# AuroraEchos/Sound-Event-Localization-and-Detection

Measured on AMD Instinct MI355X. Metric: train-step samples/sec (8ch x 128mel x 512T), higher is better.
Workload: dtype f32; 1 GPU; c3: DQSELD-TCN-S1-PHI_8ch train step, F=128 T=512 (U=L=192, SURVEY F3), batch 32/GPU, random-init weights; global_batch=32, parallelism=dp1, step_mode=graph (auto: probe 9.57 ms recorded / 12.83 ms eager per step), deterministic=True

## Files before the change

sound-event-localization-and-detection_amd/csrc/hcq_conv.hip:

```cpp
#include <string.h>
#include <type_traits>
#include "hc_common.h"

#ifndef HCQ_DBG
#define HCQ_DBG 0
#endif
#ifndef HCQ_PIN
#define HCQ_PIN 1
#endif
#ifndef HCQ_XDMA
#define HCQ_XDMA 1
#endif

namespace seld {

struct HcqP {
    const float* src;
    const float* src2;
    int nsrc;
    int mix_ytile;
    const float* wpack;
    float* dst[2];
    const float* bias[2];
    const float* addend[2];
    float* stats[2];
    int epilogue[2];
    int A;
    int N, Csrc, Cdst;
    int IB, OB;
    int W;
    int Himg;
    int dil, dpad;
    int wext;
    int nch;
    int half_src[2];
    int ytiles;
    int ob_step;
    int tile_half[3][2];
    int tile_ob[3][2];
    long long range_stride[2];
    long long ytile_stride;
    long long set_stride;
};

typedef unsigned int uintx4h __attribute__((ext_vector_type(4)));
typedef int int4h __attribute__((ext_vector_type(4)));

__device__ __forceinline__ void hcq_dma16(unsigned lds_addr, unsigned voff, int4h rsrc) {
    unsigned keep;
    asm volatile("s_mov_b32 %0, m0\n\ts_mov_b32 m0, %1\n\ts_nop 0\n\tbuffer_load_dwordx4 %2, %3, 0 offen lds\n\ts_mov_b32 m0, %0"
                 : "=&s"(keep) : "s"(lds_addr), "v"(voff), "s"(rsrc) : "memory");
}
__device__ __forceinline__ int4h hcq_rsrc(const float* base, unsigned bytes) {
    const unsigned long long a = (unsigned long long)base;
    return (int4h){(int)(unsigned)a, (int)((unsigned)(a >> 32) & 0xFFFFu), (int)bytes, 0x00020000};
}

__device__ __forceinline__ int small_div_h(int n, float inv_d) { return (int)(((float)n + 0.5f) * inv_d); }

__device__ __forceinline__ void xforms(const float b[4], float g[8]) {
    g[0] = b[1] + b[2];
    g[1] = b[0] + b[3];
    g[2] = b[0] - b[3];
    g[3] = b[1] - b[2];
    g[4] = b[2] - b[3];
    g[5] = b[1] + b[0];
    g[6] = b[2] + b[3];
    g[7] = b[1] - b[0];
}

template <int KH, int KW, int IBC, int NT1, int NT2, int NR, int XI, bool MX = false>
__global__ __launch_bounds__(256, 2) void hcq_conv_kernel(const HcqP p) {
    constexpr int TAPS = KH * KW;
    constexpr int NT = NT1 + NT2;
    constexpr int KQ = IBC * TAPS;
    constexpr int NG = (KQ + 3) / 4;
    constexpr int NPAIR = (NG + 1) / 2;
    extern __shared__ __attribute__((aligned(16))) float lds[];

    const int tid = threadIdx.x;
    const int lane = tid & 63;
    const int wave = __builtin_amdgcn_readfirstlane(tid >> 6);
    const int fr = lane & 15, fk = lane >> 4;
    const int A = p.A;
    const int ROWS = A * IBC * KH;
    const int wext = p.wext, qw = wext >> 2;
    const int buf_floats = ROWS * wext;

    const unsigned tiles_per_row = (unsigned)p.W >> 6;
    const unsigned bx = (gridDim.x & 7u) ? blockIdx.x : (blockIdx.x & 7u) * (gridDim.x >> 3) + (blockIdx.x >> 3);
    const unsigned row_g = bx / tiles_per_row;
    const int w0 = (int)(bx - row_g * tiles_per_row) * 64;
    const int n_img = (int)(row_g / (unsigned)p.Himg);
    const int h0 = (int)row_g - n_img * p.Himg;
    const int yt = blockIdx.y;
    const int set = yt >= p.ytiles ? 1 : 0;
    const int ytile = yt - set * p.ytiles;
    const bool mix_wg = ytile == p.mix_ytile;

    const unsigned S = (unsigned)(p.Himg * p.W);
    const unsigned src_bytes = (unsigned)p.N * (unsigned)p.Csrc * S * 4u;
    const unsigned OOB = 0xFFFFFFF0u;
    __amdgpu_buffer_rsrc_t rsrc = __builtin_amdgcn_make_buffer_rsrc((void*)p.src, 0, src_bytes, 0x00020000);
    unsigned xoff[XI];
    int xlds[XI];
    const unsigned xadv = (unsigned)IBC * S * 4u;
    const int total_items = ROWS * qw;
    {
        int row = small_div_h(tid, 1.0f / (float)qw);
        int quad = tid - row * qw;
        const int drow = 256 / qw, dquad = 256 - drow * qw;
        const unsigned img_base = (unsigned)n_img * (unsigned)p.Csrc * S;
#pragma unroll
        for (int i = 0; i < XI; ++i) {
            const bool in = tid + 256 * i < total_items;
            const int kh = row % KH;
            const int ci = row / KH;
            const int comp = ci / IBC;
            const int ibl = ci - comp * IBC;
            const int hh = h0 + (kh - (KH - 1) / 2);
            const int ww = w0 - p.dpad + 4 * quad;
            const bool ok = in && (unsigned)hh < (unsigned)p.Himg && (unsigned)ww < (unsigned)p.W;
            const unsigned e = img_base + ((unsigned)(comp * p.IB + ibl) * (unsigned)p.Himg + (unsigned)hh) * (unsigned)p.W + (unsigned)ww;
            xoff[i] = ok ? e * 4u : OOB;
            xlds[i] = in ? (row * qw + quad) * 4 : -1;
            row += drow;
            quad += dquad;
            if (quad >= qw) { quad -= qw; ++row; }
        }
    }
#if HCQ_XDMA
    const unsigned lds0 = (unsigned)(size_t)(__attribute__((address_space(3))) unsigned char*)lds;
    int4h xrs = hcq_rsrc(p.src, src_bytes);
    int xchunk = 0;
    int xbuf = 0;
    auto load_x = [&]() __attribute__((always_inline)) {
        if (xchunk == p.nch) {
            xrs = hcq_rsrc(p.src2, src_bytes);
#pragma unroll
            for (int i = 0; i < XI; ++i) xoff[i] = xoff[i] == OOB ? OOB : xoff[i] - (unsigned)p.nch * xadv;
        }
        ++xchunk;
        const unsigned base = lds0 + (unsigned)xbuf * (unsigned)buf_floats * 4u + 1024u * (unsigned)wave;
#pragma unroll
        for (int i = 0; i < XI; ++i) {
            if (xlds[i] >= 0) hcq_dma16(base + 4096u * (unsigned)i, xoff[i], xrs);
            xoff[i] = xoff[i] == OOB ? OOB : xoff[i] + xadv;
        }
        xbuf ^= 1;
    };
    auto store_x = [&](int) __attribute__((always_inline)) { asm volatile("s_waitcnt vmcnt(0)" ::: "memory"); };
#else
    floatx4 xr[XI];
    int xchunk = 0;
    auto load_x = [&]() __attribute__((always_inline)) {
        if (xchunk == p.nch) {
            rsrc = __builtin_amdgcn_make_buffer_rsrc((void*)p.src2, 0, src_bytes, 0x00020000);
#pragma unroll
            for (int i = 0; i < XI; ++i) xoff[i] = xoff[i] == OOB ? OOB : xoff[i] - (unsigned)p.nch * xadv;
        }
        ++xchunk;
#pragma unroll
        for (int i = 0; i < XI; ++i) {
            const uintx4h v = __builtin_amdgcn_raw_buffer_load_b128(rsrc, xoff[i], 0, 0);
            xr[i][0] = __uint_as_float(v[0]); xr[i][1] = __uint_as_float(v[1]);
            xr[i][2] = __uint_as_float(v[2]); xr[i][3] = __uint_as_float(v[3]);
            xoff[i] = xoff[i] == OOB ? OOB : xoff[i] + xadv;
        }
    };
    auto store_x = [&](int buf) __attribute__((always_inline)) {
        float* b = lds + buf * buf_floats;
#pragma unroll
        for (int i = 0; i < XI; ++i)
            if (xlds[i] >= 0) *reinterpret_cast<float4*>(b + xlds[i]) = make_float4(xr[i][0], xr[i][1], xr[i][2], xr[i][3]);
    };
#endif

    int aoff[NG];
#pragma unroll
    for (int g = 0; g < NG; ++g) {
        const int kq = (4 * g + fk) < KQ ? 4 * g + fk : 0;
        const int ibl = kq / TAPS;
        const int tap = kq - ibl * TAPS;
        const int kh = tap / KW;
        const int kw = tap - kh * KW;
        aoff[g] = (ibl * KH + kh) * wext + p.dpad + wave * 16 + fr + (kw - (KW - 1) / 2) * p.dil;
    }
    const int comp_stride = IBC * KH * wext;

    const float* wbase = p.wpack + (long long)set * p.set_stride + (long long)ytile * p.ytile_stride;
    const long long chunk_stride = p.range_stride[0] + (NR > 1 ? p.range_stride[1] : 0);

    floatx4 acc[NT][8];
#pragma unroll
    for (int t = 0; t < NT; ++t)
#pragma unroll
        for (int m = 0; m < 8; ++m) acc[t][m] = (floatx4){0.f, 0.f, 0.f, 0.f};

    float2 bfr[8][NT];
    float gm[2][8];
    float raw[4];
    constexpr int NPC = NR * NPAIR;

    bool dbg_started = false;
    auto load_b1 = [&](const float* blk, int j, int m, auto ntrc, auto t0c) __attribute__((always_inline)) {
        constexpr int NTR = decltype(ntrc)::value, T0 = decltype(t0c)::value;
        if ((HCQ_DBG & 1) && dbg_started) return;
        const float* q = blk + ((long long)(j * 8 + m) * 64 + lane) * (2 * NTR);
#pragma unroll
        for (int t = T0; t < NTR; ++t) bfr[m][t] = *reinterpret_cast<const float2*>(q + 2 * t);
    };
    auto read_raw = [&](const float* xs, int g) __attribute__((always_inline)) {
        if ((HCQ_DBG & 2) && dbg_started) return;
#pragma unroll
        for (int q = 0; q < 4; ++q) raw[q] = xs[aoff[g] + q * comp_stride];
    };
    using I0 = std::integral_constant<int, 0>;
    using INT = std::integral_constant<int, NT>;
    using INT1 = std::integral_constant<int, NT1>;
    using INT2 = std::integral_constant<int, NT2>;

    const int nchunks = p.nch * p.nsrc;
    auto kloop = [&](auto mixc) __attribute__((always_inline)) {
    constexpr bool MIX = decltype(mixc)::value;
    using IT0 = std::integral_constant<int, MIX ? NT1 : 0>;
    load_x();
    store_x(0);
#pragma unroll
    for (int m = 0; m < 8; ++m) load_b1(wbase, 0, m, INT{}, IT0{});
    __syncthreads();
    for (int ch = 0; ch < nchunks; ++ch) {
        const int buf = ch & 1;
        if (ch + 1 < nchunks && !(HCQ_DBG & 4)) load_x();
        const float* xb = lds + buf * buf_floats;
        const float* wc = wbase + (long long)ch * chunk_stride;
        const bool more = ch + 1 < nchunks;
        const float* wn = wc + chunk_stride;
        const float* xs0 = xb + p.half_src[0] * 4 * comp_stride;
        const float* xs1 = xb + p.half_src[1] * 4 * comp_stride;
        read_raw(xs0, 0);
        if (!(HCQ_DBG & 2) || !dbg_started) xforms(raw, gm[0]);
        if ((HCQ_DBG & 2) && !dbg_started) xforms(raw, gm[1]);
        dbg_started = true;
#pragma unroll
        for (int s = 0; s < NR * NG; ++s) {
            const int r = s / NG, g = s - r * NG;
            const int pc = r * NPAIR + g / 2;
            const int gst = s & 1;
            const bool last = s + 1 == NR * NG;
            const bool pair_ends = (g & 1) == 1 || g + 1 == NG;
            if (!last) {
                const int rn = (s + 1) / NG, gn = (s + 1) - rn * NG;
                read_raw(rn == 0 ? xs0 : xs1, gn);
            }
            __builtin_amdgcn_sched_barrier(0);
#pragma unroll
            for (int m = 0; m < 8; ++m) {
                if (r == 0) {
#pragma unroll
                    for (int t = MIX ? NT1 : 0; t < NT; ++t)
                        acc[t][m] = __builtin_amdgcn_mfma_f32_16x16x4f32(gm[gst][m], (g & 1) ? bfr[m][t].y : bfr[m][t].x,
                                                                          acc[t][m], 0, 0, 0);
                } else {
#pragma unroll
                    for (int t = 0; t < NT2; ++t)
                        acc[NT1 + t][m] = __builtin_amdgcn_mfma_f32_16x16x4f32(gm[gst][m], (g & 1) ? bfr[m][t].y : bfr[m][t].x,
                                                                                acc[NT1 + t][m], 0, 0, 0);
                }
                if (pair_ends) {
                    const int pn = pc + 1;
                    if (pn < NPC) {
                        const int rn = pn / NPAIR, jn = pn - rn * NPAIR;
                        if (rn == 0) load_b1(wc, jn, m, INT{}, IT0{});
                        else load_b1(wc + p.range_stride[0], jn, m, INT2{}, I0{});
                    } else if (more) {
                        load_b1(wn, 0, m, INT{}, IT0{});
                    }
                    if (HCQ_PIN && (NT >= 3 || HCQ_XDMA)) __builtin_amdgcn_sched_barrier(0);
                }
            }
            if (!last && !(HCQ_DBG & 2)) xforms(raw, gm[gst ^ 1]);
            __builtin_amdgcn_sched_barrier(0);
        }
        if (ch + 1 < nchunks && !(HCQ_DBG & 4)) store_x(buf ^ 1);
        if (!(HCQ_DBG & 8)) __syncthreads();
    }
    };
    if constexpr (MX) {
        static_assert(NR == 2 && NT1 == 1 && NT2 == 1, "the only layout with mixed-tile workgroups");
        if (mix_wg) kloop(std::true_type{});
        else kloop(std::false_type{});
    } else {
        kloop(std::false_type{});
    }

    float* const dst = p.dst[set];
    const float* const bias = p.bias[set];
    const float* const addend = p.addend[set];
    float* const stats = p.stats[set];
    const int epi = p.epilogue[set];
    const int grp = fr >> 3;
    const unsigned pos_off = (unsigned)h0 * (unsigned)p.W + (unsigned)(w0 + wave * 16 + fk * 4);
    const unsigned img_off = (unsigned)n_img * (unsigned)p.Cdst * S;
    float* redbuf = lds;
    auto epilogue = [&](auto plainc) __attribute__((always_inline)) {
        constexpr bool PLAIN = decltype(plainc)::value;
#pragma unroll
        for (int t = 0; t < NT; ++t) {
            const int ds = mix_wg ? 2 : t;
            const int ob0 = (mix_wg && t != NT1) ? -1 : p.tile_ob[ds][grp];
            const int half = p.tile_half[ds][grp];
            const bool chok = ob0 >= 0;
            const int ob = (chok ? ob0 : 0) + (mix_wg ? 0 : ytile * p.ob_step) + (fr & 7);
            floatx4 c[4];
#pragma unroll
            for (int r = 0; r < 4; ++r) {
                const float h0_ = 0.5f * acc[t][0][r], h1 = 0.5f * acc[t][1][r], h2 = 0.5f * acc[t][2][r], h3 = 0.5f * acc[t][3][r];
                c[0][r] = (h3 - h0_) + (h1 + h2) + acc[t][4][r];
                c[1][r] = (h3 - h0_) - (h1 + h2) + acc[t][5][r];
                c[2][r] = (h3 + h0_) + (h2 - h1) + acc[t][6][r];
                c[3][r] = (h3 + h0_) + (h1 - h2) - acc[t][7][r];
            }
#pragma unroll
            for (int q = 0; q < 4; ++q) {
                const int chn = (half * 4 + q) * p.OB + ob;
                const unsigned off = img_off + (unsigned)chn * S + pos_off;
                if (PLAIN) {
                    if (chok) *reinterpret_cast<float4*>(dst + off) = make_float4(c[q][0], c[q][1], c[q][2], c[q][3]);
                    continue;
                }
                float s1 = 0.f, s2 = 0.f;
                if (chok) {
                    const float bv = bias ? bias[chn] : 0.f;
                    float4 o = make_float4(c[q][0] + bv, c[q][1] + bv, c[q][2] + bv, c[q][3] + bv);
                    if (epi & SELD_EPI_ADD) {
                        const float4 ad = *reinterpret_cast<const float4*>(addend + off);
                        o.x += ad.x; o.y += ad.y; o.z += ad.z; o.w += ad.w;
                    }
                    if (epi & SELD_EPI_ACCUMULATE) {
                        const float4 old = *reinterpret_cast<const float4*>(dst + off);
                        o.x += old.x; o.y += old.y; o.z += old.z; o.w += old.w;
                    }
                    *reinterpret_cast<float4*>(dst + off) = o;
                    s1 = o.x + o.y + o.z + o.w;
                    s2 = o.x * o.x + o.y * o.y + o.z * o.z + o.w * o.w;
                }
                if (epi & SELD_EPI_STATS) {
                    s1 += __shfl_xor(s1, 16, 64);
                    s1 += __shfl_xor(s1, 32, 64);
                    s2 += __shfl_xor(s2, 16, 64);
                    s2 += __shfl_xor(s2, 32, 64);
                    if (fk == 0) {
                        const int slot = ((wave * NT + t) * 4 + q) * 16 + fr;
                        redbuf[slot * 2 + 0] = s1;
                        redbuf[slot * 2 + 1] = s2;
                    }
                }
            }
        }
    };
    if (epi == 0 && !bias) epilogue(std::true_type{});
    else epilogue(std::false_type{});
    if (epi & SELD_EPI_STATS) {
        __syncthreads();
        float* rep = stats + (size_t)(blockIdx.x % SELD_STATS_REPLICAS) * 2 * p.Cdst;
        for (int e = tid; e < NT * 4 * 16; e += 256) {
            const int fr_ = e & 15, q = (e >> 4) & 3, t = e >> 6;
            const int g_ = fr_ >> 3;
            const int ds = mix_wg ? 2 : t;
            const int ob0 = (mix_wg && t != NT1) ? -1 : p.tile_ob[ds][g_];
            if (ob0 < 0) continue;
            const int chn = (p.tile_half[ds][g_] * 4 + q) * p.OB + ob0 + (mix_wg ? 0 : ytile * p.ob_step) + (fr_ & 7);
            float a1 = 0.f, a2 = 0.f;
#pragma unroll
            for (int wv = 0; wv < 4; ++wv) {
                const int slot = ((wv * NT + t) * 4 + q) * 16 + fr_;
                a1 += redbuf[slot * 2 + 0];
                a2 += redbuf[slot * 2 + 1];
            }
            atomicAdd(rep + chn, a1);
            atomicAdd(rep + p.Cdst + chn, a2);
        }
    }
}

template <int IBC, int NT1, int NT2, int NR, int R>
__global__ __launch_bounds__(256, 2) void hcq_first_kernel(const HcqP p) {
    constexpr int KH = 3, KW = 3, TAPS = 9;
    constexpr int NT = NT1 + NT2;
    constexpr int KQ = IBC * TAPS;
    constexpr int NG = (KQ + 3) / 4;
    constexpr int NPAIR = (NG + 1) / 2;
    constexpr int NPC = NR * NPAIR;
    constexpr int XR = R + KH - 1;
    extern __shared__ __attribute__((aligned(16))) float lds[];

    const int tid = threadIdx.x;
    const int lane = tid & 63;
    const int wave = __builtin_amdgcn_readfirstlane(tid >> 6);
    const int fr = lane & 15, fk = lane >> 4;
    const int A = p.A;
    constexpr int wext = 72, qw = wext >> 2, DPAD = 4;

    const unsigned tiles_per_row = (unsigned)p.W >> 6;
    const unsigned hblocks = (unsigned)p.Himg / R;
    unsigned b = blockIdx.x;
    if ((gridDim.x & 7u) == 0) b = (blockIdx.x & 7u) * (gridDim.x >> 3) + (blockIdx.x >> 3);
    const int w0 = (int)(b % tiles_per_row) * 64;
    b /= tiles_per_row;
    const int h0 = (int)(b % hblocks) * R;
    const int n_img = (int)(b / hblocks);

    const unsigned S = (unsigned)(p.Himg * p.W);
    {
        const unsigned src_bytes = (unsigned)p.N * (unsigned)p.Csrc * S * 4u;
        const unsigned OOB = 0xFFFFFFF0u;
        const __amdgpu_buffer_rsrc_t rsrc = __builtin_amdgcn_make_buffer_rsrc((void*)p.src, 0, src_bytes, 0x00020000);
        const int items = A * IBC * XR * qw;
        const unsigned img_base = (unsigned)n_img * (unsigned)p.Csrc * S;
        constexpr float inv_qw = 1.0f / (float)qw;
        for (int f0 = tid; f0 < items; f0 += 4 * 256) {
            uintx4h v[4];
            int dst_[4];
#pragma unroll
            for (int u = 0; u < 4; ++u) {
                const int f = f0 + 256 * u;
                const int row = small_div_h(f, inv_qw);
                const int quad = f - row * qw;
                const int ci = row / XR;
                const int xr = row - ci * XR;
                const int comp = ci / IBC;
                const int ibl = ci - comp * IBC;
                const int hh = h0 - (KH - 1) / 2 + xr;
                const int ww = w0 - DPAD + 4 * quad;
                const bool ok = f < items && (unsigned)hh < (unsigned)p.Himg && (unsigned)ww < (unsigned)p.W;
                const unsigned e = img_base + ((unsigned)(comp * p.IB + ibl) * (unsigned)p.Himg + (unsigned)hh) * (unsigned)p.W + (unsigned)ww;
                v[u] = __builtin_amdgcn_raw_buffer_load_b128(rsrc, ok ? e * 4u : OOB, 0, 0);
                dst_[u] = f < items ? (row * qw + quad) * 4 : -1;
            }
#pragma unroll
            for (int u = 0; u < 4; ++u)
                if (dst_[u] >= 0)
                    *reinterpret_cast<float4*>(lds + dst_[u]) =
                        make_float4(__uint_as_float(v[u][0]), __uint_as_float(v[u][1]), __uint_as_float(v[u][2]), __uint_as_float(v[u][3]));
        }
    }
// ... 401 lines not shown
            for (int q = 0; q < 4; ++q) {
                float a1 = s1[q], a2 = s2[q];
                a1 += __shfl_xor(a1, 16, 64);
                a1 += __shfl_xor(a1, 32, 64);
                a2 += __shfl_xor(a2, 16, 64);
                a2 += __shfl_xor(a2, 32, 64);
                if (fk == 0) {
                    const int slot = ((T * 4 + wave) * 4 + q) * 16 + fr;
                    sred[slot * 2 + 0] = a1;
                    sred[slot * 2 + 1] = a2;
                }
            }
        }
    };
    tile_body(std::integral_constant<int, 0>{});
    if constexpr (NT > 1) tile_body(std::integral_constant<int, 1>{});
    if constexpr (NT > 2) tile_body(std::integral_constant<int, 2>{});

    if (want_stats) {
        __syncthreads();
        float* rep = p.stats[0] + (size_t)(blockIdx.x % SELD_STATS_REPLICAS) * 2 * p.Cdst;
        for (int e = tid; e < NT * 4 * 16; e += 256) {
            const int fr_ = e & 15, q = (e >> 4) & 3, t = e >> 6;
            const int g_ = fr_ >> 3;
            const int ob0 = p.tile_ob[t][g_];
            if (ob0 < 0) continue;
            const int chn = (p.tile_half[t][g_] * 4 + q) * p.OB + ob0 + (fr_ & 7);
            float a1 = 0.f, a2 = 0.f;
#pragma unroll
            for (int wv = 0; wv < 4; ++wv) {
                const int slot = ((t * 4 + wv) * 4 + q) * 16 + fr_;
                a1 += sred[slot * 2 + 0];
                a2 += sred[slot * 2 + 1];
            }
            atomicAdd(rep + chn, a1);
            atomicAdd(rep + p.Cdst + chn, a2);
        }
    }
}

struct HcqPackP {
    WPtrs w[2];
    float* out;
    int A, mode;
    int OA, IA, taps;
    int IBC, nch, NR, NT1, NT2, NG, NPAIR;
    int half_src[2];
    int nreg;
    int has_mix;
    int nsets;
    int nsrc;
    int ob_step;
    int tile_half[3][2], tile_ob[3][2];
    long long range_stride[2], ytile_stride, set_stride, total;
};

__device__ __forceinline__ float hcq_pack_value(const HcqPackP& p, long long idx) {
    const int NT = p.NT1 + p.NT2;
    const unsigned set_stride = (unsigned)p.set_stride, ytile_stride = (unsigned)p.ytile_stride;
    const unsigned set = (unsigned)idx / set_stride;
    unsigned r0 = (unsigned)idx - set * set_stride;
    const int ytile = (int)(r0 / ytile_stride);
    r0 -= (unsigned)ytile * ytile_stride;
    const bool mix = p.has_mix && ytile == p.nreg;
    const unsigned rs[2] = {(unsigned)p.range_stride[0], (unsigned)p.range_stride[1]};
    const unsigned chunk_stride = rs[0] + (p.NR > 1 ? rs[1] : 0);
    const int chs = (int)(r0 / chunk_stride);
    r0 -= (unsigned)chs * chunk_stride;
    const int srcsel = chs / p.nch, ch = chs - srcsel * p.nch;
    const int range = (r0 >= rs[0]) ? 1 : 0;
    if (range) r0 -= rs[0];
    const int ntr = range ? p.NT2 : NT;
    const int per_m = 64 * 2 * ntr;
    const int per_pair = 8 * per_m;
    const int j = (int)(r0 / (unsigned)per_pair);
    int r1 = (int)(r0 - (unsigned)j * (unsigned)per_pair);
    const int m = r1 / per_m;
    r1 -= m * per_m;
    const int lane = r1 / (2 * ntr);
    r1 -= lane * 2 * ntr;
    const int t = r1 >> 1, gg = r1 & 1;
    const int k = lane >> 4, n = lane & 15;
    const int g = 2 * j + gg;
    if (g >= p.NG) return 0.f;
    const int kq = 4 * g + k;
    if (kq >= p.IBC * p.taps) return 0.f;
    const int tf = range ? p.NT1 + t : t;
    const int ds = mix ? 2 : tf;
    const int grp = n >> 3;
    const int ob0 = (mix && tf != p.NT1) ? -1 : p.tile_ob[ds][grp];
    if (ob0 < 0) return 0.f;
    const int dblk = ob0 + (mix ? 0 : ytile * p.ob_step) + (n & 7);
    const int kbl = kq / p.taps;
    const int tap = kq - kbl * p.taps;
    const int sblk = ch * p.IBC + kbl;
    const int hd = p.tile_half[ds][grp], hs = p.half_src[range];
    int qsel = 0;
    if (p.A == 8) {
        if (p.mode == 0) qsel = (hd == hs) ? 0 : (hd == 1 ? 1 : -1);
        else qsel = (hd == hs) ? 0 : (hd == 0 ? 1 : -1);
    }
    if (qsel < 0) return 0.f;
    const int co = p.mode == 0 ? dblk : sblk;
    const int ci = p.mode == 0 ? sblk : dblk;
    const int tp = p.mode == 0 ? tap : p.taps - 1 - tap;
    if (co >= p.OA || ci >= p.IA) return 0.f;
    const size_t e = ((size_t)co * p.IA + ci) * p.taps + tp;
    const WPtrs& w = p.w[p.mode == 0 ? set : srcsel];
    float a[4];
#pragma unroll
    for (int c = 0; c < 4; ++c) a[c] = w.p[qsel * 4 + c][e];
    if (p.mode == 1) { a[1] = -a[1]; a[2] = -a[2]; a[3] = -a[3]; }
    switch (m) {
        case 0: return a[3] + a[1];
        case 1: return a[0] - a[2];
        case 2: return a[0] + a[2];
        case 3: return a[3] - a[1];
        case 4: return a[3] - a[2];
        case 5: return a[1] + a[0];
        case 6: return a[0] - a[1];
        default: return a[3] + a[2];
    }
}

__global__ __launch_bounds__(256) void hcq_pack_kernel(const HcqPackP p) {
    const long long idx = (long long)blockIdx.x * 256 + threadIdx.x;
    if (idx < p.total) p.out[idx] = hcq_pack_value(p, idx);
}

__global__ __launch_bounds__(256) void hcq_pack_flat_kernel(const HcqPackP* __restrict__ table, const int* __restrict__ starts,
                                                            int nentries) {
    const int b = blockIdx.x;
    int lo = 0, hi = nentries;
    while (hi - lo > 1) {
        const int mid = (lo + hi) >> 1;
        if (starts[mid] <= b) lo = mid; else hi = mid;
    }
    const HcqPackP& p = table[lo];
    const long long idx = (long long)(b - starts[lo]) * 256 + threadIdx.x;
    if (idx < p.total) p.out[idx] = hcq_pack_value(p, idx);
}

__global__ __launch_bounds__(256) void hcq_pack_table_kernel(const HcqPackP* __restrict__ table, int nentries) {
    const int e = blockIdx.y;
    if (e >= nentries) return;
    const HcqPackP& p = table[e];
    for (long long idx = (long long)blockIdx.x * 256 + threadIdx.x; idx < p.total; idx += (long long)gridDim.x * 256)
        p.out[idx] = hcq_pack_value(p, idx);
}

struct HcqPlan {
    int ok;
    int KH, KW, IBC, NT1, NT2, NR, XI, mix;
    int first_rows;
    HcqP kp;
    HcqPackP pp;
    size_t pack_floats;
    dim3 grid;
    size_t smem;
};

static HcqPlan hcq_plan(const seld_conv_desc* d, int mode, int npair) {
    HcqPlan pl{};
    const bool pool = mode == 2;
    if (pool) mode = 0;
    const int A = d->algebra;
    if (A != 4 && A != 8) return pl;
    if (d->stride[0] != 1 || d->stride[1] != 1 || d->dil[0] != 1) return pl;
    int o[2];
    hc_out_shape(d, o);
    if (o[0] != d->in[0] || o[1] != d->in[1]) return pl;
    const int KH = d->k[0], KW = d->k[1];
    if (!((KH == 1 && (KW == 1 || KW == 3)) || (KH == 3 && KW == 3))) return pl;
    if (2 * d->pad[1] != d->dil[1] * (KW - 1) || 2 * d->pad[0] != (KH - 1)) return pl;
    if (KW == 1 && d->dil[1] != 1) return pl;
    const int W = d->in[1], Himg = d->in[0];
    if (W % 64) return pl;
    const int Csrc = mode == 0 ? d->Cin : d->Cout, Cdst = mode == 0 ? d->Cout : d->Cin;
    const int IB = Csrc / A, OB = Cdst / A;
    if ((long long)d->N * Csrc * Himg * W * 4 >= 0xFFFFFFF0ll || (long long)d->N * Cdst * Himg * W * 4 >= 0xFFFFFFF0ll) return pl;
    const int taps = KH * KW;
    const int nsets = mode == 0 ? npair : 1, nsrc = mode == 1 ? npair : 1;
    const int dil = KW == 3 ? d->dil[1] : 0;
    const int dpad = KW == 3 ? (dil + 3) / 4 * 4 : 0;
    const int wext = 64 + 2 * dpad;
    static const int cand11[] = {16, 24, 8, 0}, cand13[] = {8, 4, 0}, cand33[] = {4, 2, 1, 0};
    const int* cand = taps == 1 ? cand11 : (taps == 3 ? cand13 : cand33);
    int IBC = 0;
    size_t smem = 0;
    for (int i = 0; cand[i]; ++i) {
        if (IB % cand[i]) continue;
        const int nbuf = (IB / cand[i]) * nsrc > 1 ? 2 : 1;
        const size_t need = (size_t)nbuf * A * cand[i] * KH * wext * sizeof(float);
        if (need <= 78 * 1024) { IBC = cand[i]; smem = need; break; }
    }
    if (!IBC) return pl;
    if (!pool && mode == 0 && taps == 9 && A == 8 && IB == 1 && Cdst == 192 && (long long)d->N * Himg * W >= 256 * 128 &&
        !env().conv_no_smallk) return pl;
    const int rows = A * IBC * KH;
    const int items = rows * (wext / 4);
    const int XI = (items + 255) / 256;
    if (smem < 8 * 1024) smem = 8 * 1024;
    HcqP& k = pl.kp;
    int NT1, NT2, NR, nreg, ob_step, mix = 0;
    for (int t = 0; t < 3; ++t)
        for (int g = 0; g < 2; ++g) { k.tile_half[t][g] = 0; k.tile_ob[t][g] = -1; }
    if (A == 8) {
        NR = 2;
        const int both = mode == 0 ? 1 : 0;
        const int once = 1 - both;
        k.half_src[0] = mode == 0 ? 0 : 1;
        k.half_src[1] = 1 - k.half_src[0];
        if (OB % 16 != 0 && OB % 16 != 8) return pl;
        NT1 = 1; NT2 = 1; nreg = OB / 16; ob_step = 16;
        k.tile_half[0][0] = k.tile_half[0][1] = once; k.tile_ob[0][0] = 0; k.tile_ob[0][1] = 8;
        k.tile_half[1][0] = k.tile_half[1][1] = both; k.tile_ob[1][0] = 0; k.tile_ob[1][1] = 8;
        if (OB % 16 == 8) {
            k.tile_half[2][0] = once; k.tile_ob[2][0] = OB - 8;
            k.tile_half[2][1] = both; k.tile_ob[2][1] = OB - 8;
            const long long ptiles = (long long)d->N * Himg * W / 64;
            if (OB == 24 && ptiles * nsets >= 512) { NT2 = 2; ob_step = 0; }
            else mix = 1;
        }
        if (nreg == 0) return pl;
    } else {
        NR = 1; NT2 = 0;
        k.half_src[0] = k.half_src[1] = 0;
        if (OB % 32 == 0) { NT1 = 2; nreg = OB / 32; ob_step = 32; }
        else if (OB % 16 == 0) { NT1 = 1; nreg = OB / 16; ob_step = 16; }
        else return pl;
        for (int t = 0; t < NT1; ++t) { k.tile_ob[t][0] = 16 * t; k.tile_ob[t][1] = 16 * t + 8; }
    }
    const int NG = (IBC * taps + 3) / 4, NPAIR = (NG + 1) / 2;
    const int NT = NT1 + NT2;
    k.A = A; k.N = d->N; k.Csrc = Csrc; k.Cdst = Cdst; k.IB = IB; k.OB = OB;
    k.W = W; k.Himg = Himg; k.dil = dil; k.dpad = dpad; k.wext = wext; k.nch = IB / IBC;
    k.nsrc = nsrc;
    k.ytiles = nreg + mix; k.mix_ytile = mix ? nreg : -1; k.ob_step = ob_step;
    k.range_stride[0] = (long long)NPAIR * 8 * 64 * 2 * NT;
    k.range_stride[1] = (long long)NPAIR * 8 * 64 * 2 * NT2;
    k.ytile_stride = (long long)nsrc * k.nch * (k.range_stride[0] + (NR > 1 ? k.range_stride[1] : 0));
    k.set_stride = (long long)(nreg + mix) * k.ytile_stride;
    pl.pack_floats = (size_t)k.set_stride * nsets;
    HcqPackP& q = pl.pp;
    q.A = A; q.mode = mode; q.OA = d->Cout / A; q.IA = d->Cin / A; q.taps = taps;
    q.IBC = IBC; q.nch = k.nch; q.NR = NR; q.NT1 = NT1; q.NT2 = NT2; q.NG = NG; q.NPAIR = NPAIR;
    q.half_src[0] = k.half_src[0]; q.half_src[1] = k.half_src[1];
    q.nreg = nreg; q.has_mix = mix; q.nsets = nsets; q.nsrc = nsrc; q.ob_step = ob_step;
    for (int t = 0; t < 3; ++t)
        for (int g = 0; g < 2; ++g) { q.tile_half[t][g] = k.tile_half[t][g]; q.tile_ob[t][g] = k.tile_ob[t][g]; }
    q.range_stride[0] = k.range_stride[0]; q.range_stride[1] = k.range_stride[1];
    q.ytile_stride = k.ytile_stride; q.set_stride = k.set_stride; q.total = (long long)pl.pack_floats;
    pl.KH = KH; pl.KW = KW; pl.IBC = IBC; pl.NT1 = NT1; pl.NT2 = NT2; pl.NR = NR; pl.XI = XI; pl.mix = mix;
    const long long ptot = (long long)d->N * Himg * W;
    pl.grid = dim3((unsigned)(ptot / 64), (unsigned)(k.ytiles * nsets), 1);
    pl.smem = smem;
    constexpr int FIRST_R = 8;
    if (mode == 0 && taps == 9 && IBC == IB && IB <= 2 && k.ytiles == 1 && nsets == 1 && !mix && Himg % FIRST_R == 0 && wext == 72) {
        pl.first_rows = FIRST_R;
        pl.grid = dim3((unsigned)(ptot / 64 / FIRST_R), 1, 1);
        pl.smem = ((size_t)A * IBC * (FIRST_R + 2) * wext + 4 * NT * 4 * 64 * 2) * sizeof(float);
    }
    if (pool && !pl.first_rows) return HcqPlan{};
    pl.ok = 1;
    return pl;
}

struct HcqKern { int KH, KW, IBC, NT1, NT2, NR, XI; };
static int hcq_pick(const HcqPlan& pl, HcqKern* k) {
    int xi8 = 0, xi4 = 0;
    if (pl.KH == 1 && pl.KW == 3 && pl.IBC == 8) {
        xi8 = pl.XI <= 5 ? 5 : (pl.XI <= 7 ? 7 : 9);
        xi4 = pl.XI <= 3 ? 3 : 5;
    } else if (pl.KH == 1 && pl.KW == 3 && pl.IBC == 4) { xi8 = 6; xi4 = 3; }
    else if (pl.KH == 1 && pl.KW == 1 && pl.IBC == 16) { xi8 = 8; xi4 = 4; }
    else if (pl.KH == 1 && pl.KW == 1 && pl.IBC == 24) { xi8 = 12; xi4 = 6; }
    else if (pl.KH == 1 && pl.KW == 1 && pl.IBC == 8) { xi8 = 4; xi4 = 2; }
    else if (pl.KH == 3 && pl.KW == 3 && pl.IBC == 4) { xi8 = 7; xi4 = 4; }
    else if (pl.KH == 3 && pl.KW == 3 && pl.IBC == 2) { xi8 = 4; xi4 = 2; }
    else if (pl.KH == 3 && pl.KW == 3 && pl.IBC == 1) { xi8 = 2; xi4 = 1; }
    else return 0;
    const int xi = pl.NR == 2 ? xi8 : xi4;
    if (pl.XI > xi) return 0;
    *k = HcqKern{pl.KH, pl.KW, pl.IBC, pl.NT1, pl.NT2, pl.NR, xi};
    return 1;
}

template <int KH, int KW, int IBC, int NT1, int NT2, int NR, int XI, bool MX = false>
static int hcq_launch_one(const HcqPlan& pl, hipStream_t st) {
    auto kern = hcq_conv_kernel<KH, KW, IBC, NT1, NT2, NR, XI, MX>;
    if (pl.smem > 64 * 1024 &&
        hipFuncSetAttribute((const void*)kern, hipFuncAttributeMaxDynamicSharedMemorySize, (int)pl.smem) != hipSuccess)
        return SELD_ELAUNCH;
    hipLaunchKernelGGL(kern, pl.grid, dim3(256), pl.smem, st, pl.kp);
    return check_launch();
}

template <int KH, int KW, int IBC, int XI8, int XI4>
static int hcq_launch_cfg(const HcqPlan& pl, const HcqKern& k, hipStream_t st) {
    if (k.NR == 2) {
        if (k.XI != XI8) return SELD_EUNSUPPORTED;
        if (k.NT2 == 2) return hcq_launch_one<KH, KW, IBC, 1, 2, 2, XI8>(pl, st);
        if (pl.mix) return hcq_launch_one<KH, KW, IBC, 1, 1, 2, XI8, true>(pl, st);
        return hcq_launch_one<KH, KW, IBC, 1, 1, 2, XI8>(pl, st);
    }
    if (k.XI != XI4) return SELD_EUNSUPPORTED;
    return k.NT1 == 2 ? hcq_launch_one<KH, KW, IBC, 2, 0, 1, XI4>(pl, st)
                      : hcq_launch_one<KH, KW, IBC, 1, 0, 1, XI4>(pl, st);
}

template <int IBC, int NT1, int NT2, int NR>
static int hcq_launch_first(const HcqPlan& pl, hipStream_t st) {
    auto kern = hcq_first_kernel<IBC, NT1, NT2, NR, 8>;
    if (pl.smem > 64 * 1024 &&
        hipFuncSetAttribute((const void*)kern, hipFuncAttributeMaxDynamicSharedMemorySize, (int)pl.smem) != hipSuccess)
        return SELD_ELAUNCH;
    hipLaunchKernelGGL(kern, pl.grid, dim3(256), pl.smem, st, pl.kp);
    return check_launch();
}

static bool hcq_first_takes(const HcqPlan& pl) {
    if (!pl.first_rows || pl.first_rows != 8) return false;
    if (pl.kp.epilogue[0] & ~SELD_EPI_STATS) return false;
    if (pl.NR == 2) return pl.NT1 == 1 && (pl.NT2 == 2 || pl.NT2 == 1);
    return pl.NT2 == 0 && (pl.NT1 == 1 || pl.NT1 == 2);
}

static int hcq_launch(const HcqPlan& pl, hipStream_t st) {
    HcqKern k;
    if (!hcq_pick(pl, &k)) return SELD_EUNSUPPORTED;
    if (hcq_first_takes(pl)) {
        if (k.IBC == 1) {
            if (k.NR == 2) return k.NT2 == 2 ? hcq_launch_first<1, 1, 2, 2>(pl, st) : hcq_launch_first<1, 1, 1, 2>(pl, st);
            return k.NT1 == 2 ? hcq_launch_first<1, 2, 0, 1>(pl, st) : hcq_launch_first<1, 1, 0, 1>(pl, st);
        }
        if (k.NR == 2) return k.NT2 == 2 ? hcq_launch_first<2, 1, 2, 2>(pl, st) : hcq_launch_first<2, 1, 1, 2>(pl, st);
        return k.NT1 == 2 ? hcq_launch_first<2, 2, 0, 1>(pl, st) : hcq_launch_first<2, 1, 0, 1>(pl, st);
    }
    if (k.KW == 3 && k.KH == 1 && k.IBC == 8) {
        if (k.NR == 2) {
            if (k.XI == 5) return hcq_launch_cfg<1, 3, 8, 5, 3>(pl, k, st);
            if (k.XI == 7) return hcq_launch_cfg<1, 3, 8, 7, 3>(pl, k, st);
            return hcq_launch_cfg<1, 3, 8, 9, 3>(pl, k, st);
        }
        if (k.XI == 3) return hcq_launch_cfg<1, 3, 8, 5, 3>(pl, k, st);
        return hcq_launch_cfg<1, 3, 8, 7, 5>(pl, k, st);
    }
    if (k.KH == 1 && k.KW == 3) return hcq_launch_cfg<1, 3, 4, 6, 3>(pl, k, st);
    if (k.KH == 1 && k.IBC == 16) return hcq_launch_cfg<1, 1, 16, 8, 4>(pl, k, st);
    if (k.KH == 1 && k.IBC == 24) return hcq_launch_cfg<1, 1, 24, 12, 6>(pl, k, st);
    if (k.KH == 1 && k.IBC == 8) return hcq_launch_cfg<1, 1, 8, 4, 2>(pl, k, st);
    if (k.IBC == 2) return hcq_launch_cfg<3, 3, 2, 4, 2>(pl, k, st);
    if (k.IBC == 1) return hcq_launch_cfg<3, 3, 1, 2, 1>(pl, k, st);
    return hcq_launch_cfg<3, 3, 4, 7, 4>(pl, k, st);
}

}

using namespace seld;

extern "C" size_t seld_hcq_pack_floats(const seld_conv_desc* d, int32_t mode, int32_t npair) {
    if (hc_validate(d) != SELD_OK || mode < 0 || mode > 2 || npair < 1 || npair > 2) return 0;
    if (env().conv_no_hcq) return 0;
    const HcqPlan pl = hcq_plan(d, mode, npair);
    HcqKern k;
    return (pl.ok && hcq_pick(pl, &k)) ? pl.pack_floats : 0;
}

extern "C" size_t seld_hcq_pack_entry_bytes(void) { return sizeof(HcqPackP); }

extern "C" int seld_hcq_kernel_label(const seld_conv_desc* d, int32_t mode, int32_t npair, char* buf, int32_t buflen) {
    if (hc_validate(d) != SELD_OK || !buf || buflen < 64) return SELD_EINVAL;
    const HcqPlan pl = hcq_plan(d, mode, npair);
    HcqKern k;
    if (!pl.ok || !hcq_pick(pl, &k)) return SELD_EUNSUPPORTED;
    if (mode == 2)
        snprintf(buf, buflen, "hcq_first_pool_kernel<%d, %d, %d, %d, 8>", k.IBC, k.NT1, k.NT2, k.NR);
    else if (pl.first_rows && hcq_first_takes(pl))
        snprintf(buf, buflen, "hcq_first_kernel<%d, %d, %d, %d, %d>", k.IBC, k.NT1, k.NT2, k.NR, pl.first_rows);
    else
        snprintf(buf, buflen, "hcq_conv_kernel<%d, %d, %d, %d, %d, %d, %d, %s>", k.KH, k.KW, k.IBC, k.NT1, k.NT2, k.NR, k.XI,
                 (pl.mix && k.NR == 2 && k.NT2 == 1) ? "true" : "false");
    return SELD_OK;
}

extern "C" int seld_hcq_pack_entry(const seld_conv_desc* d, int32_t mode, int32_t npair, const float* const wA[8],
                                   const float* const wB[8], float* wpack, void* entry) {
    if (hc_validate(d) != SELD_OK || !wA || !wpack || !entry) return SELD_EINVAL;
    if (mode < 0 || mode > 2 || npair < 1 || npair > 2 || (npair == 2 && !wB)) return SELD_EINVAL;
    HcqPlan pl = hcq_plan(d, mode, npair);
    if (!pl.ok) return SELD_EUNSUPPORTED;
    for (int i = 0; i < 8; ++i) {
        pl.pp.w[0].p[i] = i < d->algebra ? wA[i] : nullptr;
        pl.pp.w[1].p[i] = (npair == 2 && i < d->algebra) ? wB[i] : nullptr;
    }
    pl.pp.out = wpack;
    memcpy(entry, &pl.pp, sizeof(HcqPackP));
    return SELD_OK;
}

extern "C" int seld_hcq_pack(const seld_conv_desc* d, int32_t mode, int32_t npair, const float* const wA[8],
                             const float* const wB[8], float* wpack, void* stream) {
    HcqPackP e;
    const int rc = seld_hcq_pack_entry(d, mode, npair, wA, wB, wpack, &e);
    if (rc != SELD_OK) return rc;
    const unsigned blocks = (unsigned)((e.total + 255) / 256);
    hipLaunchKernelGGL(hcq_pack_kernel, dim3(blocks), dim3(256), 0, (hipStream_t)stream, e);
    return check_launch();
}

extern "C" int seld_hcq_pack_table(const void* table_dev, int32_t nentries, int64_t max_floats, void* stream) {
    if (!table_dev || nentries <= 0 || max_floats <= 0) return SELD_EINVAL;
    long long bx = (max_floats + 255) / 256;
    if (bx > 512) bx = 512;
    hipLaunchKernelGGL(hcq_pack_table_kernel, dim3((unsigned)bx, (unsigned)nentries), dim3(256), 0, (hipStream_t)stream,
                       (const HcqPackP*)table_dev, nentries);
    return check_launch();
}

extern "C" int seld_hcq_pack_flat(const void* table_dev, const int32_t* starts_dev, int32_t nentries, int32_t total_blocks,
                                  void* stream) {
    if (!table_dev || !starts_dev || nentries <= 0 || total_blocks <= 0) return SELD_EINVAL;
    hipLaunchKernelGGL(hcq_pack_flat_kernel, dim3((unsigned)total_blocks), dim3(256), 0, (hipStream_t)stream,
                       (const HcqPackP*)table_dev, starts_dev, nentries);
    return check_launch();
}

extern "C" int seld_hcq_conv(const seld_conv_desc* d, int32_t mode, int32_t npair, const float* x, const float* x2,
                             const float* wpack, float* const y[2], const float* const bias[2],
                             const int32_t epilogue[2], const float* const addend[2], float* const stats[2],
                             void* stream) {
    if (hc_validate(d) != SELD_OK || !x || !wpack || !y || !y[0]) return SELD_EINVAL;
    if ((mode != 0 && mode != 1) || npair < 1 || npair > 2) return SELD_EINVAL;
    if (mode == 1 && npair == 2 && !x2) return SELD_EINVAL;
    HcqPlan pl = hcq_plan(d, mode, npair);
    if (!pl.ok) return SELD_EUNSUPPORTED;
    const int nsets = mode == 0 ? npair : 1;
    for (int s = 0; s < 2; ++s) {
        const bool on = s < nsets;
        pl.kp.dst[s] = on ? y[s] : nullptr;
        pl.kp.bias[s] = (on && bias) ? bias[s] : nullptr;
        pl.kp.epilogue[s] = (on && epilogue) ? epilogue[s] : 0;
        pl.kp.addend[s] = (on && addend) ? addend[s] : nullptr;
        pl.kp.stats[s] = (on && stats) ? stats[s] : nullptr;
        if (on && !pl.kp.dst[s]) return SELD_EINVAL;
        if ((pl.kp.epilogue[s] & SELD_EPI_ADD) && !pl.kp.addend[s]) return SELD_EINVAL;
        if ((pl.kp.epilogue[s] & SELD_EPI_STATS) && !pl.kp.stats[s]) return SELD_EINVAL;
    }
    pl.kp.src = x;
    pl.kp.src2 = x2;
    pl.kp.wpack = wpack;
    return hcq_launch(pl, (hipStream_t)stream);
}


static int hcq_first_pool_impl(const seld_conv_desc* d, const float* x, const float* wpack, const float* bias,
                               int32_t want_stats, float* y, float* stats, const HcqPoolP& pp, bool fin, void* stream) {
    HcqPlan pl = hcq_plan(d, 2, 1);
    HcqKern k;
    if (!pl.ok || !hcq_pick(pl, &k) || pl.first_rows != 8) return SELD_EUNSUPPORTED;
    pl.kp.src = x; pl.kp.src2 = nullptr; pl.kp.wpack = wpack;
    pl.kp.dst[0] = y; pl.kp.bias[0] = bias; pl.kp.epilogue[0] = want_stats ? SELD_EPI_STATS : 0; pl.kp.stats[0] = stats;
    const int NT = pl.NT1 + pl.NT2;
    const int npair = ((pl.IBC * 9 + 3) / 4 + 1) / 2;
    const size_t smem = ((size_t)pl.kp.A * pl.IBC * 10 * 72 + (size_t)NT * 4 * 4 * 16 * 2 +
                         (size_t)pl.NR * npair * 8 * 64 * 2) * sizeof(float);
    hipStream_t st = (hipStream_t)stream;
#define SELD_FP(IBC_, NT1_, NT2_, NR_)                                                                                  \
    do {                                                                                                                \
        auto kern = fin ? hcq_first_pool_kernel<IBC_, NT1_, NT2_, NR_, 8, false, true>                                  \
                        : (y ? hcq_first_pool_kernel<IBC_, NT1_, NT2_, NR_, 8, true> : hcq_first_pool_kernel<IBC_, NT1_, NT2_, NR_, 8, false>); \
        if (smem > 64 * 1024 &&                                                                                         \
            hipFuncSetAttribute((const void*)kern, hipFuncAttributeMaxDynamicSharedMemorySize, (int)smem) != hipSuccess) \
            return SELD_ELAUNCH;                                                                                        \
        hipLaunchKernelGGL(kern, pl.grid, dim3(256), smem, st, pl.kp, pp);                                              \
        return check_launch();                                                                                          \
    } while (0)
    if (k.IBC == 1) {
        if (k.NR == 2) { if (k.NT2 == 2) SELD_FP(1, 1, 2, 2); else SELD_FP(1, 1, 1, 2); }
        if (k.NT1 == 2) SELD_FP(1, 2, 0, 1); else SELD_FP(1, 1, 0, 1);
    }
    if (k.NR == 2) { if (k.NT2 == 2) SELD_FP(2, 1, 2, 2); else SELD_FP(2, 1, 1, 2); }
    if (k.NT1 == 2) SELD_FP(2, 2, 0, 1); else SELD_FP(2, 1, 0, 1);
#undef SELD_FP
}

extern "C" int seld_hcq_first_pool(const seld_conv_desc* d, const float* x, const float* wpack, const float* bias,
                                   const float* gamma, int32_t want_stats, float* y, float* stats, float* pool_raw,
                                   uint8_t* idx, void* stream) {
    if (hc_validate(d) != SELD_OK || !x || !wpack || !gamma || !pool_raw || !idx || (want_stats && (!stats || !y))) return SELD_EINVAL;
    const HcqPoolP pp{gamma, pool_raw, idx, nullptr, nullptr, nullptr, nullptr, DropP{0.f, 1.f, 0, 0, nullptr}};
    return hcq_first_pool_impl(d, x, wpack, bias, want_stats, y, stats, pp, false, stream);
}

extern "C" int seld_hcq_first_pool_bn(const seld_conv_desc* d, const float* x, const float* wpack, const float* bias,
                                      const float* gamma, const float* beta, const float* mean, const float* invstd,
                                      float drop_p, uint64_t seed, uint64_t offset, const uint64_t* state, float* pool_raw,
                                      uint8_t* idx, float* out, void* stream) {
    if (hc_validate(d) != SELD_OK || !x || !wpack || !gamma || !beta || !mean || !invstd || !pool_raw || !idx || !out ||
        drop_p < 0.f || drop_p >= 1.f)
        return SELD_EINVAL;
    const HcqPoolP pp{gamma, pool_raw, idx, beta, mean, invstd, out, DropP{drop_p, 1.0f / (1.0f - drop_p), seed, offset, state}};
    return hcq_first_pool_impl(d, x, wpack, bias, 0, nullptr, nullptr, pp, true, stream);
}
```

Measured before the change: 3648 samples/s.

## Stage conv weight fragments through an LDS DMA ring instead of global loads

Adds a kring main loop that streams packed weight tiles into a double-buffered LDS ring with buffer_load...lds DMA. MFMA operands are then read from LDS instead of being fetched per lane from global memory. The planner sizes the ring as whole or half slots so workgroup occupancy is preserved, and falls back to the old global-fetch loop (GF) for A==4, KH==1 or when occupancy would drop. It also removes the non-DMA x-load path. The cost is extra LDS use, more barriers, and a more complex wait/barrier schedule.

```diff
diff --git a/sound-event-localization-and-detection_amd/csrc/hcq_conv.hip b/sound-event-localization-and-detection_amd/csrc/hcq_conv.hip
--- a/sound-event-localization-and-detection_amd/csrc/hcq_conv.hip
+++ b/sound-event-localization-and-detection_amd/csrc/hcq_conv.hip
@@ -7,9 +7,6 @@
 #endif
 #ifndef HCQ_PIN
 #define HCQ_PIN 1
-#endif
-#ifndef HCQ_XDMA
-#define HCQ_XDMA 1
 #endif
 
 namespace seld {
@@ -41,6 +38,8 @@
     long long range_stride[2];
     long long ytile_stride;
     long long set_stride;
+    int ring_off;
+    int half_slots;
 };
 
 typedef unsigned int uintx4h __attribute__((ext_vector_type(4)));
@@ -69,7 +68,7 @@
     g[7] = b[1] - b[0];
 }
 
-template <int KH, int KW, int IBC, int NT1, int NT2, int NR, int XI, bool MX = false>
+template <int KH, int KW, int IBC, int NT1, int NT2, int NR, int XI, bool MX = false, bool GF = false>
 __global__ __launch_bounds__(256, 2) void hcq_conv_kernel(const HcqP p) {
     constexpr int TAPS = KH * KW;
     constexpr int NT = NT1 + NT2;
@@ -101,7 +100,6 @@
     const unsigned S = (unsigned)(p.Himg * p.W);
     const unsigned src_bytes = (unsigned)p.N * (unsigned)p.Csrc * S * 4u;
     const unsigned OOB = 0xFFFFFFF0u;
-    __amdgpu_buffer_rsrc_t rsrc = __builtin_amdgcn_make_buffer_rsrc((void*)p.src, 0, src_bytes, 0x00020000);
     unsigned xoff[XI];
     int xlds[XI];
     const unsigned xadv = (unsigned)IBC * S * 4u;
@@ -129,7 +127,6 @@
             if (quad >= qw) { quad -= qw; ++row; }
         }
     }
-#if HCQ_XDMA
     const unsigned lds0 = (unsigned)(size_t)(__attribute__((address_space(3))) unsigned char*)lds;
     int4h xrs = hcq_rsrc(p.src, src_bytes);
     int xchunk = 0;
@@ -150,31 +147,6 @@
         xbuf ^= 1;
     };
     auto store_x = [&](int) __attribute__((always_inline)) { asm volatile("s_waitcnt vmcnt(0)" ::: "memory"); };
-#else
-    floatx4 xr[XI];
-    int xchunk = 0;
-    auto load_x = [&]() __attribute__((always_inline)) {
-        if (xchunk == p.nch) {
-            rsrc = __builtin_amdgcn_make_buffer_rsrc((void*)p.src2, 0, src_bytes, 0x00020000);
-#pragma unroll
-            for (int i = 0; i < XI; ++i) xoff[i] = xoff[i] == OOB ? OOB : xoff[i] - (unsigned)p.nch * xadv;
-        }
-        ++xchunk;
-#pragma unroll
-        for (int i = 0; i < XI; ++i) {
-            const uintx4h v = __builtin_amdgcn_raw_buffer_load_b128(rsrc, xoff[i], 0, 0);
-            xr[i][0] = __uint_as_float(v[0]); xr[i][1] = __uint_as_float(v[1]);
-            xr[i][2] = __uint_as_float(v[2]); xr[i][3] = __uint_as_float(v[3]);
-            xoff[i] = xoff[i] == OOB ? OOB : xoff[i] + xadv;
-        }
-    };
-    auto store_x = [&](int buf) __attribute__((always_inline)) {
-        float* b = lds + buf * buf_floats;
-#pragma unroll
-        for (int i = 0; i < XI; ++i)
-            if (xlds[i] >= 0) *reinterpret_cast<float4*>(b + xlds[i]) = make_float4(xr[i][0], xr[i][1], xr[i][2], xr[i][3]);
-    };
-#endif
 
     int aoff[NG];
 #pragma unroll
@@ -276,7 +248,7 @@
                     } else if (more) {
                         load_b1(wn, 0, m, INT{}, IT0{});
                     }
-                    if (HCQ_PIN && (NT >= 3 || HCQ_XDMA)) __builtin_amdgcn_sched_barrier(0);
+                    if (HCQ_PIN) __builtin_amdgcn_sched_barrier(0);
                 }
             }
             if (!last && !(HCQ_DBG & 2)) xforms(raw, gm[gst ^ 1]);
@@ -285,13 +257,143 @@
         if (ch + 1 < nchunks && !(HCQ_DBG & 4)) store_x(buf ^ 1);
         if (!(HCQ_DBG & 8)) __syncthreads();
     }
+    };
+
+    auto kring = [&](auto mixc) __attribute__((always_inline)) {
+    constexpr bool MIX = decltype(mixc)::value;
+    const bool half = p.half_slots != 0;
+    const unsigned tile_bytes = half ? 2048u : 4096u;
+    const unsigned slot_bytes = tile_bytes * NT;
+    const unsigned ring0 = lds0 + (unsigned)p.ring_off;
+    const float* const ringf = lds + (p.ring_off >> 2);
+    const int4h frs = hcq_rsrc(wbase, (unsigned)p.ytile_stride * 4u);
+    unsigned foff = 1024u * (unsigned)wave + 16u * (unsigned)lane;
+    unsigned fslot = 0;
+    unsigned rslot = 0;
+    bool freq = false;
+    const bool xfull = 256 * (XI - 1) + 64 * wave < total_items;
+    auto load_f = [&](auto ntrc) __attribute__((always_inline)) {
+        constexpr int NTRn = decltype(ntrc)::value;
+        const unsigned nbytes = tile_bytes * NTRn;
+        if (!((HCQ_DBG & 1) && freq)) {
+            const unsigned dst = ring0 + fslot * slot_bytes + 1024u * (unsigned)wave;
+#pragma unroll
+            for (int i = 0; i < NTRn; ++i)
+                if (4096u * i + 1024u * (unsigned)wave < nbytes) hcq_dma16(dst + 4096u * i, foff + 4096u * i, frs);
+        }
+        freq = true;
+        foff += nbytes;
+        fslot ^= 1u;
+    };
+    auto open_unit = [&](bool counted) __attribute__((always_inline)) {
+        if (counted) asm volatile("s_waitcnt vmcnt(%0)" :: "n"(XI) : "memory");
+        else asm volatile("s_waitcnt vmcnt(0)" ::: "memory");
+        if (HCQ_DBG & 8) return;
+        asm volatile("s_waitcnt lgkmcnt(0)\n\ts_barrier" ::: "memory");
+    };
+    float ga[8], gb[8];
+    float2 fb[3][NT];
+    load_x();
+    load_f(INT{});
+    bool dbg_raw = false;
+    for (int ch = 0; ch < nchunks; ++ch) {
+        const bool more = ch + 1 < nchunks;
+        const float* xb = lds + (ch & 1) * buf_floats;
+        const float* xs0 = xb + p.half_src[0] * 4 * comp_stride;
+        const float* xs1 = xb + p.half_src[1] * 4 * comp_stride;
+        bool xreq = false;
+#pragma unroll
+        for (int pc = 0; pc < NPC; ++pc) {
+            const int r = pc / NPAIR, j = pc - r * NPAIR;
+            const int g0 = 2 * j;
+            const bool two = g0 + 1 < NG;
+            const int ntr = r == 0 ? NT : NT2;
+            const int t0 = (r == 0 && MIX) ? NT1 : 0;
+            const int ab = r == 0 ? 0 : NT1;
+            auto request_next_pair = [&]() __attribute__((always_inline)) {
+                if (pc + 1 < NPC) {
+                    if ((pc + 1) / NPAIR == 0) load_f(INT{});
+                    else load_f(INT2{});
+                } else if (more) {
+                    load_f(INT{});
+                }
+            };
+            open_unit(pc == 1 && !half && xreq && xfull);
+            if (half) {
+                if (r == 0) load_f(INT{});
+                else load_f(INT2{});
+            } else {
+                request_next_pair();
+            }
+            if (pc == 0 && more && !((HCQ_DBG & 4) && ch > 0)) { load_x(); xreq = true; }
+            const float* fsl = ringf + rslot * (slot_bytes >> 2);
+            auto read_form = [&](int idx, int st) __attribute__((always_inline)) {
+                const float2* q = reinterpret_cast<const float2*>(fsl) + (idx * 64 + lane) * ntr;
+#pragma unroll
+                for (int t = 0; t < NT; ++t)
+                    if (t >= t0 && t < ntr) fb[st][t] = q[t];
+            };
+            read_form(0, 0);
+            read_form(1, 1);
+            if (!((HCQ_DBG & 2) && dbg_raw)) {
+                float ra[4], rb[4];
+                const float* xs = r == 0 ? xs0 : xs1;
+#pragma unroll
+                for (int q = 0; q < 4; ++q) ra[q] = xs[aoff[g0] + q * comp_stride];
+                if (two) {
+#pragma unroll
+                    for (int q = 0; q < 4; ++q) rb[q] = xs[aoff[two ? g0 + 1 : g0] + q * comp_stride];
+                }
+                xforms(ra, ga);
+                if (two) xforms(rb, gb);
+                dbg_raw = true;
+            }
+            __builtin_amdgcn_sched_barrier(0);
+#pragma unroll
+            for (int m = 0; m < 8; ++m) {
+                if (m == 4 && half) {
+                    open_unit(pc == 0 && xreq && xfull);
+                    request_next_pair();
+                    rslot ^= 1u;
+                    fsl = ringf + rslot * (slot_bytes >> 2);
+                    read_form(0, 4 % 3);
+                    read_form(1, 5 % 3);
+                }
+                if (m + 2 < 8) {
+                    if (m + 2 < 4 || m >= 4) read_form(half ? (m + 2) & 3 : m + 2, (m + 2) % 3);
+                    else if (!half) read_form(m + 2, (m + 2) % 3);
+                }
+                __builtin_amdgcn_sched_barrier(0);
+#pragma unroll
+                for (int t = 0; t < NT; ++t)
+                    if (t >= t0 && t < ntr)
+                        acc[ab + t][m] = __builtin_amdgcn_mfma_f32_16x16x4f32(ga[m], fb[m % 3][t].x, acc[ab + t][m], 0, 0, 0);
+                if (two) {
+#pragma unroll
+                    for (int t = 0; t < NT; ++t)
+                        if (t >= t0 && t < ntr)
+                            acc[ab + t][m] = __builtin_amdgcn_mfma_f32_16x16x4f32(gb[m], fb[m % 3][t].y, acc[ab + t][m], 0, 0, 0);
+                }
+                __builtin_amdgcn_sched_barrier(0);
+            }
+            rslot ^= 1u;
+            if (HCQ_DBG & 1) rslot = 0;
+        }
+    }
+    if (p.epilogue[set] & SELD_EPI_STATS) __syncthreads();
     };
     if constexpr (MX) {
         static_assert(NR == 2 && NT1 == 1 && NT2 == 1, "the only layout with mixed-tile workgroups");
-        if (mix_wg) kloop(std::true_type{});
-        else kloop(std::false_type{});
+        if constexpr (GF) {
+            if (mix_wg) kloop(std::true_type{});
+            else kloop(std::false_type{});
+        } else {
+            if (mix_wg) kring(std::true_type{});
+            else kring(std::false_type{});
+        }
     } else {
-        kloop(std::false_type{});
+        if constexpr (GF) kloop(std::false_type{});
+        else kring(std::false_type{});
     }
 
     float* const dst = p.dst[set];
@@ -999,6 +1101,7 @@
 struct HcqPlan {
     int ok;
     int KH, KW, IBC, NT1, NT2, NR, XI, mix;
+    int gf;
     int first_rows;
     HcqP kp;
     HcqPackP pp;
@@ -1044,10 +1147,6 @@
     if (!IBC) return pl;
     if (!pool && mode == 0 && taps == 9 && A == 8 && IB == 1 && Cdst == 192 && (long long)d->N * Himg * W >= 256 * 128 &&
         !env().conv_no_smallk) return pl;
-    const int rows = A * IBC * KH;
-    const int items = rows * (wext / 4);
-    const int XI = (items + 255) / 256;
-    if (smem < 8 * 1024) smem = 8 * 1024;
     HcqP& k = pl.kp;
     int NT1, NT2, NR, nreg, ob_step, mix = 0;
     for (int t = 0; t < 3; ++t)
@@ -1078,8 +1177,27 @@
         else return pl;
         for (int t = 0; t < NT1; ++t) { k.tile_ob[t][0] = 16 * t; k.tile_ob[t][1] = 16 * t + 8; }
     }
+    const int NT = NT1 + NT2;
+    int half_slots = 0;
+    bool gf = A == 4 && KH == 1;
+    if (!pool && !gf) {
+        const auto wgs = [](size_t bytes) { const size_t n = (size_t)160 * 1024 / (bytes < 8192 ? 8192 : bytes); return n > 3 ? (size_t)3 : n; };
+        const size_t wgs0 = wgs(smem);
+        const size_t whole = (size_t)2 * 4096 * NT, halves = (size_t)2 * 2048 * NT;
+        if (wgs(smem + whole) >= wgs0 || (mix && wgs(smem + whole) >= 2)) half_slots = 0;
+        else if (wgs(smem + halves) >= wgs0 || KH != 1) half_slots = 1;
+        else gf = true;
+        if (!gf) {
+            k.ring_off = (int)smem;
+            k.half_slots = half_slots;
+            smem += half_slots ? halves : whole;
+        }
+    }
+    const int rows = A * IBC * KH;
+    const int items = rows * (wext / 4);
+    const int XI = (items + 255) / 256;
+    if (smem < 8 * 1024) smem = 8 * 1024;
     const int NG = (IBC * taps + 3) / 4, NPAIR = (NG + 1) / 2;
-    const int NT = NT1 + NT2;
     k.A = A; k.N = d->N; k.Csrc = Csrc; k.Cdst = Cdst; k.IB = IB; k.OB = OB;
     k.W = W; k.Himg = Himg; k.dil = dil; k.dpad = dpad; k.wext = wext; k.nch = IB / IBC;
     k.nsrc = nsrc;
@@ -1099,6 +1217,7 @@
     q.range_stride[0] = k.range_stride[0]; q.range_stride[1] = k.range_stride[1];
     q.ytile_stride = k.ytile_stride; q.set_stride = k.set_stride; q.total = (long long)pl.pack_floats;
     pl.KH = KH; pl.KW = KW; pl.IBC = IBC; pl.NT1 = NT1; pl.NT2 = NT2; pl.NR = NR; pl.XI = XI; pl.mix = mix;
+    pl.gf = gf ? 1 : 0;
     const long long ptot = (long long)d->N * Himg * W;
     pl.grid = dim3((unsigned)(ptot / 64), (unsigned)(k.ytiles * nsets), 1);
     pl.smem = smem;
@@ -1133,9 +1252,9 @@
     return 1;
 }
 
-template <int KH, int KW, int IBC, int NT1, int NT2, int NR, int XI, bool MX = false>
+template <int KH, int KW, int IBC, int NT1, int NT2, int NR, int XI, bool MX = false, bool GF = false>
 static int hcq_launch_one(const HcqPlan& pl, hipStream_t st) {
-    auto kern = hcq_conv_kernel<KH, KW, IBC, NT1, NT2, NR, XI, MX>;
+    auto kern = hcq_conv_kernel<KH, KW, IBC, NT1, NT2, NR, XI, MX, GF>;
     if (pl.smem > 64 * 1024 &&
         hipFuncSetAttribute((const void*)kern, hipFuncAttributeMaxDynamicSharedMemorySize, (int)pl.smem) != hipSuccess)
         return SELD_ELAUNCH;
@@ -1147,11 +1266,23 @@
 static int hcq_launch_cfg(const HcqPlan& pl, const HcqKern& k, hipStream_t st) {
     if (k.NR == 2) {
         if (k.XI != XI8) return SELD_EUNSUPPORTED;
+        if constexpr (KH == 1) {
+            if (pl.gf) {
+                if (k.NT2 == 2) return hcq_launch_one<KH, KW, IBC, 1, 2, 2, XI8, false, true>(pl, st);
+                if (pl.mix) return hcq_launch_one<KH, KW, IBC, 1, 1, 2, XI8, true, true>(pl, st);
+                return hcq_launch_one<KH, KW, IBC, 1, 1, 2, XI8, false, true>(pl, st);
+            }
+        }
         if (k.NT2 == 2) return hcq_launch_one<KH, KW, IBC, 1, 2, 2, XI8>(pl, st);
         if (pl.mix) return hcq_launch_one<KH, KW, IBC, 1, 1, 2, XI8, true>(pl, st);
         return hcq_launch_one<KH, KW, IBC, 1, 1, 2, XI8>(pl, st);
     }
     if (k.XI != XI4) return SELD_EUNSUPPORTED;
+    if constexpr (KH == 1) {
+        if (pl.gf)
+            return k.NT1 == 2 ? hcq_launch_one<KH, KW, IBC, 2, 0, 1, XI4, false, true>(pl, st)
+                              : hcq_launch_one<KH, KW, IBC, 1, 0, 1, XI4, false, true>(pl, st);
+    }
     return k.NT1 == 2 ? hcq_launch_one<KH, KW, IBC, 2, 0, 1, XI4>(pl, st)
                       : hcq_launch_one<KH, KW, IBC, 1, 0, 1, XI4>(pl, st);
 }
@@ -1226,8 +1357,8 @@
     else if (pl.first_rows && hcq_first_takes(pl))
         snprintf(buf, buflen, "hcq_first_kernel<%d, %d, %d, %d, %d>", k.IBC, k.NT1, k.NT2, k.NR, pl.first_rows);
     else
-        snprintf(buf, buflen, "hcq_conv_kernel<%d, %d, %d, %d, %d, %d, %d, %s>", k.KH, k.KW, k.IBC, k.NT1, k.NT2, k.NR, k.XI,
-                 (pl.mix && k.NR == 2 && k.NT2 == 1) ? "true" : "false");
+        snprintf(buf, buflen, "hcq_conv_kernel<%d, %d, %d, %d, %d, %d, %d, %s, %s>", k.KH, k.KW, k.IBC, k.NT1, k.NT2, k.NR, k.XI,
+                 (pl.mix && k.NR == 2 && k.NT2 == 1) ? "true" : "false", pl.gf ? "true" : "false");
     return SELD_OK;
 }
 
```

Result: faster. 3757 samples/s, median of 6 (+3.0%).
